# 0xPolygonZero/plonky2

Hardware: NVIDIA H100
Metric: goldilocks_field_elements_per_s_ntt_lde_merkle (higher is better)
Workload: dtype u64

## Files before the change

plonky2_b200/csrc/gl_poseidon.cuh:

```cuda
#pragma once
#include "gl_field.cuh"
#include "gl_poseidon_constants.h"

#if !defined(GL_MDS_INT) && !defined(GL_MDS_FP64)
#define GL_MDS_FP64 1
#endif
#if defined(GL_MDS_FP64) && (defined(__CUDA_ARCH__) || defined(GL_FP64_ON_HOST))
#define GL_FP64_PATH 1
#endif
#if defined(GL_FP64_PATH) && !defined(GL_PARTIAL_FAST)
#define GL_PARTIAL_F64 1
#endif

namespace gl {

struct PoseidonTables {
    uint64_t rc[360];
    uint64_t fast_first[12];
    uint64_t fast_rc[22];
    uint64_t vs[22 * 11];
    uint64_t w_hats[22 * 11];
    uint64_t init[11 * 11];
    uint64_t zeros[12];
    uint32_t mds_circ[12];
    uint32_t mds_00;
    uint32_t pad_;
    double mds_f64[13];
    double nrc_f64[9][24];
    double nrcs_f64[9][24];
    double pks_f64[11][24];
    double pan_f64[11][2];
};

#if defined(__CUDACC__)
__constant__ PoseidonTables c_pos;
#endif

inline const PoseidonTables& host_poseidon_tables() {
    static PoseidonTables t = [] {
        PoseidonTables x;
        for (int i = 0; i < 360; i++) x.rc[i] = GL_POSEIDON_RC[i];
        for (int i = 0; i < 12; i++) x.fast_first[i] = GL_POSEIDON_FAST_FIRST_RC[i];
        for (int i = 0; i < 22; i++) x.fast_rc[i] = GL_POSEIDON_FAST_RC[i];
        for (int i = 0; i < 242; i++) x.vs[i] = GL_POSEIDON_FAST_VS[i];
        for (int i = 0; i < 242; i++) x.w_hats[i] = GL_POSEIDON_FAST_W_HATS[i];
        for (int i = 0; i < 121; i++) x.init[i] = GL_POSEIDON_FAST_INIT_MATRIX[i];
        for (int i = 0; i < 12; i++) x.zeros[i] = 0;
        for (int i = 0; i < 12; i++) x.mds_circ[i] = (uint32_t)GL_POSEIDON_MDS_CIRC[i];
        x.mds_00 = (uint32_t)(GL_POSEIDON_MDS_CIRC[0] + GL_POSEIDON_MDS_DIAG[0]);
        x.pad_ = 0;
        for (int i = 0; i < 12; i++) x.mds_f64[i] = (double)GL_POSEIDON_MDS_CIRC[i];
        x.mds_f64[12] = (double)(GL_POSEIDON_MDS_CIRC[0] + GL_POSEIDON_MDS_DIAG[0]);
        for (int r = 0; r < 9; r++) {
            const uint64_t* src = (r < 3) ? &x.rc[12 * (r + 1)] : (r == 3) ? x.fast_first
                                : (r < 7) ? &x.rc[12 * (r + 23)] : (r == 7) ? x.zeros : &x.rc[48];
            for (int i = 0; i < 12; i++) {
                x.nrc_f64[r][2 * i] = (double)(uint32_t)src[i];
                x.nrc_f64[r][2 * i + 1] = (double)(uint32_t)(src[i] >> 32);
            }
            const double b2[2] = {4398046511104.0 + 1024.0, 4398046511104.0 - 2048.0};
            for (int q = 0; q < 6; q++)
                for (int l = 0; l < 2; l++) {
                    const double k0 = x.nrc_f64[r][2 * q + l] + b2[l], k6 = x.nrc_f64[r][2 * (q + 6) + l] + b2[l];
                    x.nrcs_f64[r][12 * l + q] = (k0 + k6) * 0.5;
                    x.nrcs_f64[r][12 * l + 6 + q] = (k0 - k6) * 0.5;
                }
        }
        const double bl = 1125899906842624.0 + 262144.0, bh = 1125899906842624.0 - 524288.0;
        uint64_t M[12][12];
        for (int i = 0; i < 12; i++)
            for (int j = 0; j < 12; j++)
                M[i][j] = GL_POSEIDON_MDS_CIRC[(j - i + 12) % 12] + ((i == 0 && j == 0) ? GL_POSEIDON_MDS_DIAG[0] : 0);
        for (int pr = 0; pr < 11; pr++) {
            const uint64_t* cA = &x.rc[12 * (5 + 2 * pr)];
            const uint64_t* cB = &x.rc[12 * (5 + 2 * pr + 1)];
            x.pan_f64[pr][0] = (double)(uint32_t)cA[0];
            x.pan_f64[pr][1] = (double)(uint32_t)(cA[0] >> 32);
            double k2[12][2];
            for (int i = 0; i < 12; i++) {
                unsigned __int128 k = cB[i];
                for (int t = 0; t < 12; t++) k += (unsigned __int128)M[i][t] * cA[t];
                const unsigned __int128 PP = (unsigned __int128)0xFFFFFFFF00000001ULL;
                if (i == 0) k += 8 * (PP - cA[0] % PP);
                const uint64_t kr = (uint64_t)(k % PP);
                const bool biased = (i == 0) || (pr == 10);
                k2[i][0] = (double)(uint32_t)kr + (biased ? bl : 0.0);
                k2[i][1] = (double)(uint32_t)(kr >> 32) + (biased ? bh : 0.0);
            }
            for (int q = 0; q < 6; q++)
                for (int l = 0; l < 2; l++) {
                    x.pks_f64[pr][12 * l + q] = (k2[q][l] + k2[q + 6][l]) * 0.5;
                    x.pks_f64[pr][12 * l + 6 + q] = (k2[q][l] - k2[q + 6][l]) * 0.5;
                }
        }
        return x;
    }();
    return t;
}

#if defined(__CUDA_ARCH__)
#define GL_POS (c_pos)
#else
#define GL_POS (host_poseidon_tables())
#endif

struct Acc160 {
    uint64_t lo, hi;
    uint32_t top;
};
GL_HD void acc_mul(Acc160& a, uint64_t x, uint64_t y) {
    uint64_t pl, ph;
    mul_wide(x, y, pl, ph);
#if defined(__CUDA_ARCH__)
    asm("add.cc.u64 %0, %0, %3;\n\taddc.cc.u64 %1, %1, %4;\n\taddc.u32 %2, %2, 0;"
        : "+l"(a.lo), "+l"(a.hi), "+r"(a.top)
        : "l"(pl), "l"(ph));
#else
    unsigned __int128 s = (unsigned __int128)a.lo + pl;
    a.lo = (uint64_t)s;
    unsigned __int128 h = (unsigned __int128)a.hi + ph + (uint64_t)(s >> 64);
    a.hi = (uint64_t)h;
    a.top += (uint32_t)(h >> 64);
#endif
}
GL_HD uint64_t acc_reduce(const Acc160& a) {
    uint64_t r = reduce128(a.lo, a.hi);
    return sub(r, (uint64_t)a.top << 32);
}

GL_HD constexpr uint32_t mds_entry(int i, int j) {
    constexpr uint32_t circ[12] = {17, 15, 41, 16, 2, 28, 13, 13, 39, 18, 34, 20};
    return circ[(j - i + 12) % 12] + ((i == 0 && j == 0) ? 8u : 0u);
}

struct MdsCirc {
    static GL_HD constexpr double c(int d) {
        constexpr double circ[12] = {17, 15, 41, 16, 2, 28, 13, 13, 39, 18, 34, 20};
        return circ[((d % 12) + 12) % 12];
    }
};
struct MdsCirc2 {
    static GL_HD constexpr double c(int d) {
        double a = 0;
        for (int t = 0; t < 12; t++) a += MdsCirc::c(t) * MdsCirc::c(d - t);
        return a;
    }
};
template <class K>
GL_HD constexpr double circ_half_p(int k) { return (K::c(k) + K::c(k + 6)) * 0.5; }
template <class K>
GL_HD constexpr double circ_half_m(int k) { return (K::c(k) - K::c(k + 6)) * 0.5; }

#if !defined(GL_F64_TRACK)
#define GL_F64_TRACK(x)
#endif
#if defined(GL_FP64_PATH)
GL_HD double f64_fma(double a, double b, double c) {
#if defined(__CUDA_ARCH__)
    return fma(a, b, c);
#else
    return __builtin_fma(a, b, c);
#endif
}
GL_HD double u32_to_f64(uint32_t x) {
#if defined(__CUDA_ARCH__) && defined(GL_CVT_MAGIC)
    return __hiloint2double(0x43300000, (int)x) - 4503599627370496.0;
#else
    return (double)x;
#endif
}
GL_HD double u32_magic_f64(uint32_t x) {
#if defined(__CUDA_ARCH__)
    return __hiloint2double(0x43300000, (int)x);
#else
    const uint64_t b = 0x4330000000000000ULL | x;
    double d;
    __builtin_memcpy(&d, &b, 8);
    return d;
#endif
}
GL_HD uint64_t f64_pair_to_u64(double al, double ah) {
#if defined(__CUDA_ARCH__) && !defined(GL_CVT_MAGIC)
    const uint64_t ul = __double2ull_rz(al), uh = __double2ull_rz(ah);
    uint32_t r1, r2;
    asm("add.cc.u32 %0, %2, %3;\n\taddc.u32 %1, %4, 0;" : "=r"(r1), "=r"(r2) : "r"(hi32(ul)), "r"(lo32(uh)), "r"(hi32(uh)));
    return reduce96(pack64(lo32(ul), r1), r2);
#elif defined(__CUDA_ARCH__)
    const double bl = al + 4503599627370496.0, bh = ah + 4503599627370496.0;
    const uint32_t al0 = (uint32_t)__double2loint(bl), al1 = (uint32_t)__double2hiint(bl) & 0xFFFFFu;
    const uint32_t ah0 = (uint32_t)__double2loint(bh), ah1 = (uint32_t)__double2hiint(bh) & 0xFFFFFu;
    uint32_t r1, r2;
    asm("add.cc.u32 %0, %2, %3;\n\taddc.u32 %1, %4, 0;" : "=r"(r1), "=r"(r2) : "r"(al1), "r"(ah0), "r"(ah1));
    return reduce96(pack64(al0, r1), r2);
#else
    const unsigned __int128 v = (unsigned __int128)(uint64_t)al + ((unsigned __int128)(uint64_t)ah << 32);
    return reduce96((uint64_t)v, (uint32_t)(v >> 64));
#endif
}
template <class K>
GL_HD void circ12_f64(const double v[12], const double* seed, double out[12]) {
    double vp[6], vm[6];
#pragma unroll
    for (int j = 0; j < 6; j++) {
        vp[j] = v[j] + v[j + 6];
        vm[j] = v[j] - v[j + 6];
    }
#pragma unroll
    for (int r = 0; r < 6; r++) {
        double sp = seed[r], sm = seed[6 + r];
#pragma unroll
        for (int j = 0; j < 6; j++) {
            sp = f64_fma(vp[j], circ_half_p<K>((j - r + 6) % 6), sp);
            sm = f64_fma(vm[j], j >= r ? circ_half_m<K>(j - r) : -circ_half_m<K>(j - r + 6), sm);
        }
        GL_F64_TRACK(sp);
        GL_F64_TRACK(sm);
        out[r] = sp + sm;
        out[r + 6] = sp - sm;
    }
}
#endif

GL_HD uint64_t sbox7(uint64_t x) {
    uint64_t x2 = sqr(x);
    uint64_t x4 = sqr(x2);
    uint64_t x3 = mul(x, x2);
    return mul(x3, x4);
}

#if defined(GL_FP64_PATH)
GL_HD void sbox7_f64(uint64_t x, double& L, double& H) {
#if defined(GL_SBOX_SQR4)
    const uint64_t x2 = sqr(x);
    const uint64_t x4 = sqr(x2);
#else
    const uint64_t x2 = sqr_3w(x);
    const uint64_t x4 = sqr_3w(x2);
#endif
    const uint64_t x3 = mul(x, x2);
    uint64_t lo, hi;
    mul_wide(x3, x4, lo, hi);
#if !defined(GL_SBOX_I2F)
    const double m0 = u32_magic_f64((uint32_t)lo), m1 = u32_magic_f64((uint32_t)(lo >> 32));
    const double m2 = u32_magic_f64((uint32_t)hi), m3 = u32_magic_f64((uint32_t)(hi >> 32));
    H = (m1 - 9007199254740992.0) + m2;
    L = (m0 - m2) - (m3 - 4503599627370496.0);
#else
    const double d0 = u32_to_f64((uint32_t)lo), d1 = u32_to_f64((uint32_t)(lo >> 32));
    const double d2 = u32_to_f64((uint32_t)hi), d3 = u32_to_f64((uint32_t)(hi >> 32));
    L = (d0 - d2) - d3;
    H = d1 + d2;
#endif
}
#endif

GL_HD void mds_layer_add(uint64_t s[12], const uint64_t* nrc, const double* nrcd = nullptr) {
    (void)nrcd;
    const PoseidonTables& T = GL_POS;
#if defined(GL_FP64_PATH)
    {
        double dl[12], dh[12];
#pragma unroll
        for (int i = 0; i < 12; i++) {
            dl[i] = u32_to_f64((uint32_t)s[i]);
            dh[i] = u32_to_f64((uint32_t)(s[i] >> 32));
        }
#pragma unroll
        for (int r = 0; r < 12; r++) {
            double al, ah;
            if (nrcd) {
                al = nrcd[2 * r];
                ah = nrcd[2 * r + 1];
            } else {
                const uint64_t c = nrc[r];
                al = u32_to_f64((uint32_t)c);
                ah = u32_to_f64((uint32_t)(c >> 32));
            }
#pragma unroll
            for (int i = 0; i < 12; i++) {
                const double m = (r == 0 && i == 0) ? T.mds_f64[12] : T.mds_f64[i];
                al = f64_fma(dl[(i + r) % 12], m, al);
                ah = f64_fma(dh[(i + r) % 12], m, ah);
            }
            s[r] = f64_pair_to_u64(al, ah);
        }
    }
#else
    uint32_t lo[12], hi[12];
#pragma unroll
    for (int i = 0; i < 12; i++) {
        lo[i] = (uint32_t)s[i];
        hi[i] = (uint32_t)(s[i] >> 32);
    }
#pragma unroll
    for (int r = 0; r < 12; r++) {
        const uint64_t c = nrc[r];
        uint64_t al = (uint32_t)c, ah = c >> 32;
#pragma unroll
        for (int i = 0; i < 12; i++) {
            const uint32_t m = (r == 0 && i == 0) ? T.mds_00 : T.mds_circ[i];
#if defined(__CUDA_ARCH__)
            asm("mad.wide.u32 %0, %1, %2, %0;" : "+l"(al) : "r"(lo[(i + r) % 12]), "r"(m));
            asm("mad.wide.u32 %0, %1, %2, %0;" : "+l"(ah) : "r"(hi[(i + r) % 12]), "r"(m));
#else
            al += (uint64_t)lo[(i + r) % 12] * m;
            ah += (uint64_t)hi[(i + r) % 12] * m;
#endif
        }
#if defined(__CUDA_ARCH__)
        uint32_t r1, r2;
        asm("add.cc.u32 %0, %2, %3;\n\taddc.u32 %1, %4, 0;"
            : "=r"(r1), "=r"(r2)
            : "r"(hi32(al)), "r"(lo32(ah)), "r"(hi32(ah)));
        s[r] = reduce96(pack64(lo32(al), r1), r2);
#else
        uint64_t l64 = al + (ah << 32);
        uint32_t h32 = (uint32_t)(ah >> 32) + (l64 < al ? 1u : 0u);
        s[r] = reduce96(l64, h32);
#endif
    }
#endif
}
GL_HD void mds_layer(uint64_t s[12]) { mds_layer_add(s, GL_POS.zeros); }

GL_HD void full_round_fused(uint64_t s[12], const uint64_t* next_rc, const double* next_rcd = nullptr) {
#pragma unroll
    for (int i = 0; i < 12; i++) s[i] = sbox7(s[i]);
    mds_layer_add(s, next_rc, next_rcd);
}
#if defined(GL_FP64_PATH)
GL_HD void full_round_f64(uint64_t s[12], const double* rcs) {
    double dl[12], dh[12];
#pragma unroll
    for (int i = 0; i < 12; i++) sbox7_f64(s[i], dl[i], dh[i]);
    double ol[12], oh[12];
    circ12_f64<MdsCirc>(dl, rcs, ol);
    ol[0] = f64_fma(dl[0], 8.0, ol[0]);
    circ12_f64<MdsCirc>(dh, rcs + 12, oh);
    oh[0] = f64_fma(dh[0], 8.0, oh[0]);
#pragma unroll
    for (int r = 0; r < 12; r++) {
        GL_F64_TRACK(ol[r]);
        GL_F64_TRACK(oh[r]);
        s[r] = f64_pair_to_u64(ol[r], oh[r]);
    }
}
#endif
GL_HD void full_round(uint64_t s[12], const uint64_t* rc) {
#pragma unroll
    for (int i = 0; i < 12; i++) s[i] = add_canonical(s[i], rc[i]);
    full_round_fused(s, GL_POS.zeros);
}

GL_HD void poseidon_partial_rounds_noconst(uint64_t s[12]) {
    const PoseidonTables& T = GL_POS;
    {
        uint64_t res[11];
#pragma unroll 1
        for (int c = 0; c < 11; c++) {
            Acc160 a = {0, 0, 0};
#pragma unroll
            for (int r = 1; r < 12; r++) acc_mul(a, s[r], T.init[(r - 1) * 11 + c]);
            res[c] = acc_reduce(a);
        }
#pragma unroll
        for (int i = 1; i < 12; i++) s[i] = res[i - 1];
    }
#pragma unroll 1
    for (int r = 0; r < 22; r++) {
        uint64_t s0 = add_canonical(sbox7(s[0]), T.fast_rc[r]);
        Acc160 a = {0, 0, 0};
        acc_mul(a, s0, T.mds_00);
#pragma unroll
        for (int i = 1; i < 12; i++) acc_mul(a, s[i], T.w_hats[r * 11 + i - 1]);
#pragma unroll
        for (int i = 1; i < 12; i++) s[i] = mul_add(s0, T.vs[r * 11 + i - 1], s[i]);
        s[0] = acc_reduce(a);
    }
}
#if defined(GL_FP64_PATH)
GL_HD void poseidon_partial_rounds_f64(uint64_t s[12]) {
    const PoseidonTables& T = GL_POS;
    double L[12], H[12];
#pragma unroll
    for (int i = 1; i < 12; i++) {
        L[i] = u32_to_f64((uint32_t)s[i]);
        H[i] = u32_to_f64((uint32_t)(s[i] >> 32));
    }
    uint64_t s0 = s[0];
#pragma unroll 1
    for (int rp = 0; rp < 11; rp++) {
        sbox7_f64(s0, L[0], H[0]);
        double aL = T.pan_f64[rp][0], aH = T.pan_f64[rp][1];
#pragma unroll
        for (int j = 0; j < 12; j++) {
            aL = f64_fma(L[j], (double)mds_entry(0, j), aL);
            aH = f64_fma(H[j], (double)mds_entry(0, j), aH);
        }
        double zL, zH;
        sbox7_f64(f64_pair_to_u64(aL + (1125899906842624.0 + 262144.0), aH + (1125899906842624.0 - 524288.0)), zL, zH);
        zL -= aL;
        zH -= aH;
        const double* k = T.pks_f64[rp];
        {
            double n[12];
            circ12_f64<MdsCirc2>(L, k, n);
#pragma unroll
            for (int i = 0; i < 12; i++) {
                n[i] = f64_fma(L[0], 8.0 * MdsCirc::c(12 - i), n[i]);
                n[i] = f64_fma(zL, (double)mds_entry(i, 0), n[i]);
            }
            n[0] = f64_fma(aL, 8.0, n[0]);
#pragma unroll
            for (int i = 0; i < 12; i++) {
                L[i] = n[i];
                GL_F64_TRACK(n[i]);
            }
        }
        {
            double n[12];
            circ12_f64<MdsCirc2>(H, k + 12, n);
#pragma unroll
            for (int i = 0; i < 12; i++) {
                n[i] = f64_fma(H[0], 8.0 * MdsCirc::c(12 - i), n[i]);
                n[i] = f64_fma(zH, (double)mds_entry(i, 0), n[i]);
            }
            n[0] = f64_fma(aH, 8.0, n[0]);
#pragma unroll
            for (int i = 0; i < 12; i++) {
                H[i] = n[i];
                GL_F64_TRACK(n[i]);
            }
        }
        s0 = f64_pair_to_u64(L[0], H[0]);
        if (rp != 10) {
            const double C84 = 29014219670751100192948224.0;
            const double I32 = 2.3283064365386962890625e-10;
#pragma unroll
            for (int i = 1; i < 12; i++) {
                const double th = (H[i] + C84) - C84;
                const double hlo = H[i] - th;
                const double l2 = f64_fma(th, -I32, L[i]);
                const double tl = (l2 + C84) - C84;
                L[i] = l2 - tl;
                H[i] = f64_fma(tl, I32, f64_fma(th, I32, hlo));
            }
        }
    }
    s[0] = s0;
#pragma unroll
    for (int i = 1; i < 12; i++) s[i] = f64_pair_to_u64(L[i], H[i]);
}
#endif

GL_HD void poseidon_partial_rounds(uint64_t s[12]) {
#pragma unroll
    for (int i = 0; i < 12; i++) s[i] = add_canonical(s[i], GL_POS.fast_first[i]);
    poseidon_partial_rounds_noconst(s);
}

template <bool SYNC = false>
GL_HD void poseidon_permute_t(uint64_t s[12]) {
    const PoseidonTables& T = GL_POS;
#pragma unroll
    for (int i = 0; i < 12; i++) s[i] = add_canonical(s[i], T.rc[i]);
#pragma unroll 1
    for (int r = 0; r < 8; r++) {
#if defined(GL_PARTIAL_F64)
        const uint64_t* nrc = (r < 3) ? &T.rc[12 * (r + 1)] : (r == 3) ? &T.rc[48]
                            : (r < 7) ? &T.rc[12 * (r + 23)] : T.zeros;
        (void)nrc;
        full_round_f64(s, T.nrcs_f64[r == 3 ? 8 : r]);
#else
        const uint64_t* nrc = (r < 3) ? &T.rc[12 * (r + 1)] : (r == 3) ? T.fast_first
                            : (r < 7) ? &T.rc[12 * (r + 23)] : T.zeros;
        full_round_fused(s, nrc, T.nrc_f64[r]);
#endif
#if defined(__CUDA_ARCH__)
        if (SYNC) __syncthreads();
#endif
        if (r == 3) {
#if defined(GL_PARTIAL_F64)
            poseidon_partial_rounds_f64(s);
#else
            poseidon_partial_rounds_noconst(s);
#pragma unroll
            for (int i = 0; i < 12; i++) s[i] = add_canonical(s[i], T.rc[12 * 26 + i]);
#endif
        }
    }
}
GL_HD void poseidon_permute(uint64_t s[12]) { poseidon_permute_t<false>(s); }

template <bool SYNC = false>
GL_HD void two_to_one(const uint64_t l[4], const uint64_t r[4], uint64_t out[4]) {
    uint64_t s[12] = {l[0], l[1], l[2], l[3], r[0], r[1], r[2], r[3], 0, 0, 0, 0};
    poseidon_permute_t<SYNC>(s);
#pragma unroll
    for (int i = 0; i < 4; i++) out[i] = canon(s[i]);
}

template <bool NOOP_SHORT = true, bool SYNC = false>
GL_HD void hash_or_noop_strided(const uint64_t* in, size_t stride, uint32_t W, uint64_t out[4]) {
    if (NOOP_SHORT && W <= 4) {
#pragma unroll
        for (uint32_t i = 0; i < 4; i++) out[i] = (i < W) ? canon(in[i * stride]) : 0;
        return;
    }
    uint64_t s[12];
#pragma unroll
    for (int i = 0; i < 12; i++) s[i] = 0;
    for (uint32_t off = 0; off < W; off += 8) {
#pragma unroll
        for (uint32_t i = 0; i < 8; i++)
            if (off + i < W) s[i] = in[(size_t)(off + i) * stride];
        poseidon_permute_t<SYNC>(s);
    }
#pragma unroll
    for (int i = 0; i < 4; i++) out[i] = canon(s[i]);
}

}
```

Baseline: 7.787 billion.

## Defer partial-round constants and use integer-bit renormalization in FP64 Poseidon

Reformulates the FP64 partial-round pair so that most round constants are carried as a host-precomputed deferred offset. Only a scalar constant is seeded into the circulant, and a final correction is added after the loop. The per-limb renormalization also replaces the four-add C84 rounding trick with a magic-number integer bit manipulation, and the mds column update is folded into a single FMA per element. This cuts the FP64 and FMA instruction count in the partial-round loop. The cost is more complex host-side constant derivation and new precision assumptions about limb ranges.

```diff
diff --git a/plonky2_b200/csrc/gl_poseidon.cuh b/plonky2_b200/csrc/gl_poseidon.cuh
--- a/plonky2_b200/csrc/gl_poseidon.cuh
+++ b/plonky2_b200/csrc/gl_poseidon.cuh
@@ -30,6 +30,9 @@
     double nrcs_f64[9][24];
     double pks_f64[11][24];
     double pan_f64[11][2];
+    double pk0_f64[11][2];
+    double pad_f64[11][2];
+    double pdf_f64[22];
 };
 
 #if defined(__CUDACC__)
@@ -71,27 +74,57 @@
         for (int i = 0; i < 12; i++)
             for (int j = 0; j < 12; j++)
                 M[i][j] = GL_POSEIDON_MDS_CIRC[(j - i + 12) % 12] + ((i == 0 && j == 0) ? GL_POSEIDON_MDS_DIAG[0] : 0);
+        const unsigned __int128 PP = (unsigned __int128)0xFFFFFFFF00000001ULL;
+        uint64_t CC[12][12];
+        for (int i = 0; i < 12; i++)
+            for (int j = 0; j < 12; j++) {
+                CC[i][j] = 0;
+                for (int t = 0; t < 12; t++) CC[i][j] += GL_POSEIDON_MDS_CIRC[(t - i + 12) % 12] * GL_POSEIDON_MDS_CIRC[(j - t + 12) % 12];
+            }
+        uint64_t d[12] = {0};
         for (int pr = 0; pr < 11; pr++) {
             const uint64_t* cA = &x.rc[12 * (5 + 2 * pr)];
             const uint64_t* cB = &x.rc[12 * (5 + 2 * pr + 1)];
             x.pan_f64[pr][0] = (double)(uint32_t)cA[0];
             x.pan_f64[pr][1] = (double)(uint32_t)(cA[0] >> 32);
             double k2[12][2];
+            uint64_t k2r[12];
             for (int i = 0; i < 12; i++) {
                 unsigned __int128 k = cB[i];
                 for (int t = 0; t < 12; t++) k += (unsigned __int128)M[i][t] * cA[t];
-                const unsigned __int128 PP = (unsigned __int128)0xFFFFFFFF00000001ULL;
                 if (i == 0) k += 8 * (PP - cA[0] % PP);
                 const uint64_t kr = (uint64_t)(k % PP);
+                k2r[i] = kr;
                 const bool biased = (i == 0) || (pr == 10);
                 k2[i][0] = (double)(uint32_t)kr + (biased ? bl : 0.0);
                 k2[i][1] = (double)(uint32_t)(kr >> 32) + (biased ? bh : 0.0);
+            }
+            {
+                unsigned __int128 a = cA[0];
+                for (int t = 0; t < 12; t++) a += (unsigned __int128)M[0][t] * d[t];
+                const uint64_t ar = (uint64_t)(a % PP);
+                x.pad_f64[pr][0] = (double)(uint32_t)ar;
+                x.pad_f64[pr][1] = (double)(uint32_t)(ar >> 32);
+                uint64_t e[12];
+                for (int i = 0; i < 12; i++) {
+                    unsigned __int128 v = k2r[i];
+                    for (int t = 0; t < 12; t++) v += (unsigned __int128)CC[i][t] * d[t];
+                    e[i] = (uint64_t)(v % PP);
+                }
+                x.pk0_f64[pr][0] = ((double)(uint32_t)e[0] + bl) * 0.5;
+                x.pk0_f64[pr][1] = ((double)(uint32_t)(e[0] >> 32) + bh) * 0.5;
+                d[0] = 0;
+                for (int i = 1; i < 12; i++) d[i] = e[i];
             }
             for (int q = 0; q < 6; q++)
                 for (int l = 0; l < 2; l++) {
                     x.pks_f64[pr][12 * l + q] = (k2[q][l] + k2[q + 6][l]) * 0.5;
                     x.pks_f64[pr][12 * l + 6 + q] = (k2[q][l] - k2[q + 6][l]) * 0.5;
                 }
+        }
+        for (int i = 1; i < 12; i++) {
+            x.pdf_f64[2 * (i - 1)] = (double)(uint32_t)d[i] + bl;
+            x.pdf_f64[2 * (i - 1) + 1] = (double)(uint32_t)(d[i] >> 32) + bh;
         }
         return x;
     }();
@@ -174,6 +207,33 @@
     return __hiloint2double(0x43300000, (int)x);
 #else
     const uint64_t b = 0x4330000000000000ULL | x;
+    double d;
+    __builtin_memcpy(&d, &b, 8);
+    return d;
+#endif
+}
+GL_HD uint32_t f64_lo_word(double x) {
+#if defined(__CUDA_ARCH__)
+    return (uint32_t)__double2loint(x);
+#else
+    uint64_t b;
+    __builtin_memcpy(&b, &x, 8);
+    return (uint32_t)b;
+#endif
+}
+GL_HD uint32_t f64_hi_word(double x) {
+#if defined(__CUDA_ARCH__)
+    return (uint32_t)__double2hiint(x);
+#else
+    uint64_t b;
+    __builtin_memcpy(&b, &x, 8);
+    return (uint32_t)(b >> 32);
+#endif
+}
+GL_HD double f64_from_bits(uint64_t b) {
+#if defined(__CUDA_ARCH__)
+    return __longlong_as_double((long long)b);
+#else
     double d;
     __builtin_memcpy(&d, &b, 8);
     return d;
@@ -379,6 +439,54 @@
     }
 }
 #if defined(GL_FP64_PATH)
+GL_HD void partial_pair_limbs(double v[12], const double* k, double z, double a) {
+    const double x0 = v[0];
+    double n[12];
+#if defined(GL_PAIR_RENORM_F64)
+    circ12_f64<MdsCirc2>(v, k, n);
+#else
+    const double seed[12] = {k[0], 0, 0, 0, 0, 0, k[0], 0, 0, 0, 0, 0};
+    circ12_f64<MdsCirc2>(v, seed, n);
+#endif
+#if defined(GL_PAIR_RENORM_F64)
+    const double za = z - a;
+#pragma unroll
+    for (int i = 0; i < 12; i++) {
+        n[i] = f64_fma(x0, 8.0 * MdsCirc::c(12 - i), n[i]);
+        n[i] = f64_fma(za, (double)mds_entry(i, 0), n[i]);
+    }
+    n[0] = f64_fma(a, 8.0, n[0]);
+#else
+    const double w = f64_fma(x0, 8.0, z - a);
+#pragma unroll
+    for (int i = 0; i < 12; i++) n[i] = f64_fma(w, MdsCirc::c(12 - i), n[i]);
+    n[0] = f64_fma(z, 8.0, n[0]);
+#endif
+#pragma unroll
+    for (int i = 0; i < 12; i++) {
+        v[i] = n[i];
+        GL_F64_TRACK(n[i]);
+    }
+}
+GL_HD void partial_pair_renorm(double& L, double& H) {
+#if defined(GL_PAIR_RENORM_F64)
+    const double C84 = 29014219670751100192948224.0;
+    const double I32 = 2.3283064365386962890625e-10;
+    const double th = (H + C84) - C84;
+    const double hlo = H - th;
+    const double l2 = f64_fma(th, -I32, L);
+    const double tl = (l2 + C84) - C84;
+    L = l2 - tl;
+    H = f64_fma(tl, I32, f64_fma(th, I32, hlo));
+#else
+    const double tL = L + 6755399441055744.0, tH = H + 6755399441055744.0;
+    const uint32_t rL = f64_lo_word(tL), hL = f64_hi_word(tL), rH = f64_lo_word(tH), hH = f64_hi_word(tH);
+    const uint64_t yl = (0x4330000143300000ULL + rL) - hH;
+    const uint64_t yh = 0x4330000000000000ULL + rH + hL + hH;
+    L = f64_from_bits(yl) - 4503603921813504.0;
+    H = f64_from_bits(yh) - 4503601882857472.0;
+#endif
+}
 GL_HD void poseidon_partial_rounds_f64(uint64_t s[12]) {
     const PoseidonTables& T = GL_POS;
     double L[12], H[12];
@@ -391,7 +499,11 @@
 #pragma unroll 1
     for (int rp = 0; rp < 11; rp++) {
         sbox7_f64(s0, L[0], H[0]);
+#if defined(GL_PAIR_RENORM_F64)
         double aL = T.pan_f64[rp][0], aH = T.pan_f64[rp][1];
+#else
+        double aL = T.pad_f64[rp][0], aH = T.pad_f64[rp][1];
+#endif
 #pragma unroll
         for (int j = 0; j < 12; j++) {
             aL = f64_fma(L[j], (double)mds_entry(0, j), aL);
@@ -399,55 +511,30 @@
         }
         double zL, zH;
         sbox7_f64(f64_pair_to_u64(aL + (1125899906842624.0 + 262144.0), aH + (1125899906842624.0 - 524288.0)), zL, zH);
-        zL -= aL;
-        zH -= aH;
+#if defined(GL_PAIR_RENORM_F64)
         const double* k = T.pks_f64[rp];
-        {
-            double n[12];
-            circ12_f64<MdsCirc2>(L, k, n);
-#pragma unroll
-            for (int i = 0; i < 12; i++) {
-                n[i] = f64_fma(L[0], 8.0 * MdsCirc::c(12 - i), n[i]);
-                n[i] = f64_fma(zL, (double)mds_entry(i, 0), n[i]);
-            }
-            n[0] = f64_fma(aL, 8.0, n[0]);
-#pragma unroll
-            for (int i = 0; i < 12; i++) {
-                L[i] = n[i];
-                GL_F64_TRACK(n[i]);
-            }
-        }
-        {
-            double n[12];
-            circ12_f64<MdsCirc2>(H, k + 12, n);
-#pragma unroll
-            for (int i = 0; i < 12; i++) {
-                n[i] = f64_fma(H[0], 8.0 * MdsCirc::c(12 - i), n[i]);
-                n[i] = f64_fma(zH, (double)mds_entry(i, 0), n[i]);
-            }
-            n[0] = f64_fma(aH, 8.0, n[0]);
-#pragma unroll
-            for (int i = 0; i < 12; i++) {
-                H[i] = n[i];
-                GL_F64_TRACK(n[i]);
-            }
-        }
+        partial_pair_limbs(L, k, zL, aL);
+        partial_pair_limbs(H, k + 12, zH, aH);
+#else
+        partial_pair_limbs(L, &T.pk0_f64[rp][0], zL, aL);
+        partial_pair_limbs(H, &T.pk0_f64[rp][1], zH, aH);
+#endif
         s0 = f64_pair_to_u64(L[0], H[0]);
         if (rp != 10) {
-            const double C84 = 29014219670751100192948224.0;
-            const double I32 = 2.3283064365386962890625e-10;
-#pragma unroll
-            for (int i = 1; i < 12; i++) {
-                const double th = (H[i] + C84) - C84;
-                const double hlo = H[i] - th;
-                const double l2 = f64_fma(th, -I32, L[i]);
-                const double tl = (l2 + C84) - C84;
-                L[i] = l2 - tl;
-                H[i] = f64_fma(tl, I32, f64_fma(th, I32, hlo));
-            }
+#pragma unroll
+            for (int i = 1; i < 12; i++) partial_pair_renorm(L[i], H[i]);
         }
     }
     s[0] = s0;
+#if !defined(GL_PAIR_RENORM_F64)
+#pragma unroll
+    for (int i = 1; i < 12; i++) {
+        L[i] += T.pdf_f64[2 * (i - 1)];
+        H[i] += T.pdf_f64[2 * (i - 1) + 1];
+        GL_F64_TRACK(L[i]);
+        GL_F64_TRACK(H[i]);
+    }
+#endif
 #pragma unroll
     for (int i = 1; i < 12; i++) s[i] = f64_pair_to_u64(L[i], H[i]);
 }
```

Result: faster. 8.050 billion (median of 6 runs) (+3.4%).
